# ArtoriasAbyssslayer/HashModNFFBanks-IDR

Hardware: AMD Instinct MI355X
Metric: rays/sec fwd+bwd (hash+SDF MLP) (higher is better)
Workload: dtype f32; 1 GPU; DTU-shaped synthetic uniform-sphere rays, MultiResHash L=16 T=2^19 F=2 (BASELINE.json configs[1]), full IDR training step (forward + IDRLoss + backward + clip + Adam), weights held at the geometric initialisation (lr = 0): the SURVEY.md 8(d) workload; grid_config=C2, rays_per_gpu=2048, global_rays=2048, parallelism=single GPU, world=1, ranks_seen=1, step=HIP-graph captured static-shape step

## Files before the change

hashmodnffbanks_idr_amd/_lib.py:

```python
import ctypes as C
import os

import torch

_PKG = os.path.dirname(os.path.abspath(__file__))
LIB_PATH = os.environ.get("HM_LIB_PATH") or os.path.join(_PKG, "libhashmod.so")
_lib = None

_p = C.c_void_p
_i64 = C.c_int64
_int = C.c_int

SIGNATURES = {
    "hm_version": (_int, []),
    "hm_last_error": (C.c_char_p, []),
    "hm_device_count": (_int, []),
    "hm_grid_desc_create": (_int, [_int, _int, _p, _p, _p, C.POINTER(_p)]),
    "hm_grid_desc_destroy": (None, [_p]),
    "hm_grid_embed_dim": (_int, [_p]),
    "hm_corner_ids": (_int, [_p, _int, _p, _i64, _p, _p, _p]),
    "hm_diag_gather_calib": (_int, [_p, _i64, _i64, _int, _int, _p, _p]),
    "hm_diag_mfma_f32_stream": (_int, [_int, _int, _p, _p]),
    "hm_encode_fwd": (_int, [_p, _p, _i64, _p, _p, _p, _i64, _int, _p]),
    "hm_encode_workspace_bytes": (_i64, [_p, _i64]),
# ... 2 lines not shown
    "hm_encode_bwd_workspace_bytes": (_i64, [_p, _i64]),
    "hm_encode_bwd_table_ws": (_int, [_p, _p, _i64, _p, _i64, _p, _int, _p, _i64, _p]),
    "hm_encode_rows": (_int, [_p, _p, _i64, _int, _p, _p, _p]),
    "hm_encode_bwd_table_sorted": (_int, [_p, _p, _p, _i64, _int, _p, _i64, _p, _p, _p]),
    "hm_sort_workspace_bytes": (_i64, [_i64]),
    "hm_sort_pairs_i32": (_int, [_p, _i64, _int, _p, _p, _p, _i64, _p]),
    "hm_encode_bwd_input": (_int, [_p, _p, _i64, _p, _p, _i64, _p, _p, _p]),
    "hm_encode_jvp": (_int, [_p, _p, _i64, _p, _p, _p, _i64, _p]),
    "hm_encode_bwd_table_jvp": (_int, [_p, _p, _i64, _p, _p, _i64, _p, _p]),
    "hm_fourier_bwd_input": (_int, [_p, _i64, _p, _int, _p, _i64, _p, _p]),
    "hm_fourier_bwd_input_bwd": (_int, [_p, _i64, _p, _int, _p, _i64, _p, _p, _p, _i64, _int, _p]),
    "hm_weight_norm_multi": (_int, [_int, _int, _p, _p]),
    "hm_rownorm": (_int, [_int, _p, _p, _p, _p, _p, _i64, _int, C.c_float, _p]),
    "hm_sine": (_int, [_int, _p, _p, _p, _p, _p, _i64, C.c_float, _p]),
    "hm_posenc": (_int, [_int, _p, _int, _int, _p, _i64, _p, _i64, _p, _p, _i64, _p, _i64, _p]),
    "hm_sdf_fwd": (_int, [_p, _p, _p, _i64, _p, _p, _p, _i64, _int, _int, _int, _p, _int, _p]),
    "hm_nffb_fwd": (_int, [_p, _p, _p, _i64, _p, _p, _p, _i64, _int, _p, _p]),
    "hm_sdf_fwd_emb": (_int, [_p, _p, _i64, _int, _i64, _p, _i64, _int, _int, _p, _int, _p]),
    "hm_sdf_net_fits": (_int, [_p, _int, _int]),
    "hm_diag_sdf_lds": (_int, [_p, _int, _int, _int, _p]),
    "hm_trace_workspace_bytes": (_i64, [_i64, _p]),
    "hm_trace_guard_clear": (_int, [_p, _i64, _p]),
    "hm_trace_guard_tolerances": (_int, [_p, _p]),
    "hm_trace_forward": (_int, [_p, _p, _p, _p, _int, _int, _p, _p, _p, _p, _p, _p, _i64, _i64, _p, _p, _p, _p, _p, _p,
                                _i64, _p, _p]),
    "hm_trace_workspace_bytes_nffb": (_i64, [_i64, _p, _int]),
    "hm_trace_forward_nffb": (_int, [_p, _p, _p, _p, _p, _int, _int, _p, _p, _p, _p, _p, _p, _i64, _i64, _p, _p, _p, _p,
                                     _p, _p, _i64, _p, _p]),
    "hm_pack_mlp_layer_bf16": (_int, [_p, _i64, _int, _int, _int, _p, _p]),
    "hm_sdf_fwd_bf16": (_int, [_p, _p, _p, _i64, _p, _p, _p, _i64, _int, _p, _i64, _p]),
    "hm_sdf_fwd_emb_bf16": (_int, [_p, _p, _i64, _int, _i64, _p, _i64, _p, _i64, _p]),
    "hm_pack_mlp_layer_split": (_int, [_p, _i64, _int, _int, _int, C.c_float, C.c_float, _int, _p, _p]),
    "hm_sdf_fwd_split": (_int, [_p, _p, _p, _i64, _p, _p, _p, _i64, _int, _p, _i64, _p]),
    "hm_sdf_fwd_emb_split": (_int, [_p, _p, _i64, _int, _i64, _p, _i64, _p, _i64, _p]),
    "hm_pack_mlp_layers": (_int, [_p, _int, _p]),
    "hm_pack_mlp_layer": (_int, [_p, _i64, _p, _int, _int, _int, _p, _p, _p, _p]),
    "hm_softplus": (_int, [_int, _p, _p, _p, _p, _p, _i64, C.c_float, C.c_float, _p]),
    "hm_sdf_head": (_int, [_int, _p, _i64, _i64, C.c_float, _p, _p, _p, _p, _p, _p]),
    "hm_colsum": (_int, [_p, _i64, _i64, _i64, _p, _p]),
    "hm_colsum_acc": (_int, [_p, _i64, _i64, _i64, _p, _p]),
    "hm_colsum_acc_multi": (_int, [_p, _int, _p]),
    "hm_copy2d_f32": (_int, [_p, _i64, _p, _i64, _i64, _i64, _p]),
    "hm_camera_rays": (_int, [_p, _p, _p, _i64, _i64, C.c_float, _p, _p, _p, _p, _p]),
    "hm_idr_loss": (_int, [_p, _p, _p, _p, _p, _i64, _p, _i64, C.c_float, C.c_float, C.c_float, _p, _p, _p, _p, _p]),
    "hm_idr_loss_dev": (_int, [_p, _p, _p, _p, _p, _i64, _p, _i64, _p, _p, _p, _p, _p, _p]),
    "hm_adam_scratch_floats": (_i64, [_p, _int]),
# ... 243 lines not shown
```

hashmodnffbanks_idr_amd/csrc/hm_sdf.hip:

```cpp
#include "hm_common.h"

#include <math.h>
#include <stdlib.h>

namespace {

#include "hm_sdf_common.h"
#include "hm_trace_dev.h"

#ifdef HM_SDF_PHASE_PROBE
__device__ unsigned long long hm_probe_ts[128];
#define HM_PROBE(i_)                                                                                  \
    do {                                                                                              \
        if (blockIdx.x == 0 && threadIdx.x == 0 && it == 1 && (i_) < 120) hm_probe_ts[(i_)] = wall_clock64(); \
        if (blockIdx.x == 0 && threadIdx.x == 0 && it == 1 && ((i_) == 0 || (i_) == 100))                 \
            hm_probe_ts[120 + ((i_) != 0)] = clock64();         \
    } while (0)
#define HM_PROBE_WAVES(base_)                                                                                  \
    do {                                                                                                       \
        if (blockIdx.x == 0 && (threadIdx.x & 63) == 0 && it == 1 && li == 2) hm_probe_ts[(base_) + (threadIdx.x >> 6)] = wall_clock64(); \
    } while (0)
#define HM_PROBE_S(i_)                                                                                \
    do {                                                                                              \
        if (blockIdx.x == 0 && threadIdx.x == 0 && (i_) < 120) hm_probe_ts[(i_)] = wall_clock64();   \
    } while (0)
#else
#define HM_PROBE(i_) do { } while (0)
#define HM_PROBE_WAVES(base_) do { } while (0)
#define HM_PROBE_S(i_) do { } while (0)
#endif

#include "hm_sdf_tile64.h"
#include "hm_sdf_split_tile.h"

__host__ __device__ inline SdfLds sdf_lds_small(const SdfNet &net, int E, int pts) {
    return sdf_lds(pts, 2, net.x_groups * pts * 4, 1, (E + 15) / 16 * 4 * pts * 4, kWaves);
}

template <int FRAC>
__global__ __launch_bounds__(kThreadsSdf, 2) void sdf_fwd_kernel(HmLevels lv, SdfNet net,
                                                                  const float *__restrict__ x, int64_t n,
                                                                  const float *__restrict__ table,
                                                                  const float *__restrict__ Bf,
                                                                  float *__restrict__ out, int64_t out_stride,
                                                                  int out_cols, const int32_t *__restrict__ n_dev, int64_t run_min,
                                                                  int64_t run_max, SdfFillArgs fa) {
    extern __shared__ __align__(16) float lds[];
    if (n_dev) n = min(n, (int64_t)max(*n_dev, 0));
    if (n < run_min || n > run_max) return;
    SdfFill fb = {nullptr, nullptr, 0, 0};
    if (fa.n_dev) {
        fb.x = fa.x;
        fb.out = fa.out;
        fb.n = max(*fa.n_dev, 0);
        if (fa.prev_dev)
            fb.tile0 = fill_quota(max(*fa.prev_dev, 0), fa.prev_grid, (fb.n + kPts - 1) / kPts, run_min);
// ... 400 lines not shown
                                                                          float *__restrict__ scan_out, int c_scan,
                                                                          int64_t scan_cap, int64_t scan_min,
                                                                          int64_t scan_hide, int c_prev1, int grid1,
                                                                          int c_prev2, int grid2) {
    extern __shared__ __align__(16) float lds[];
    const int64_t n_scan = min((int64_t)max(a.w.cnt[c_scan], 0), scan_cap);
    const int64_t n_sec = a.w.cnt[C_NSEC];
    if (n_sec > 0 && n_iters > 0) {
        const int pts = a.w.cnt[C_NSEL_PTS] >= scan_hide ? 16 : (n_sec <= m4_max ? 4 : (n_sec <= m8_max ? 8 : 16));
        secant_role<FRAC>(lv, net, table, Bf, a, n_iters, n_sec, pts, lds);
    }
    if (n_scan < scan_min) return;
    const int64_t tb = (n_scan + kPts - 1) / kPts;
    int64_t done = c_prev1 >= 0 ? fill_quota(max(a.w.cnt[c_prev1], 0), grid1, tb, scan_min) : 0;
    if (c_prev2 >= 0) done += fill_quota(max(a.w.cnt[c_prev2], 0), grid2, tb - done, scan_min);
    const int64_t skip = done * kPts;
    if (skip >= n_scan) return;
    const SdfFill none = {nullptr, nullptr, 0, 0};
    sdf64_run<FRAC, true>(lv, net, scan_x + skip * 3, n_scan - skip, table, Bf, scan_out + skip, 1, 1, lds,
                          reinterpret_cast<unsigned *>(a.w.cnt + C_TILE_CURSOR), none);
}

template <int KIND, int FRAC>
__global__ __launch_bounds__(kThreadsSdf, 2) void sdf_refine_scan_kernel(HmLevels lv, SdfNet net, SdfNet net_split,
                                                                          const float *__restrict__ table,
                                                                          const float *__restrict__ Bf, TraceArgs a,
                                                                          int c_ref, int64_t scan_off, int64_t scan_min) {
    extern __shared__ __align__(16) float lds[];
    __shared__ unsigned s_scan_tile;
    const int64_t n_ref = min((int64_t)max(a.w.cnt[c_ref], 0), a.w.cap);
    const int64_t n_scan = min((int64_t)max(a.w.cnt[C_NSEL_PTS], 0), a.w.cap);
    if (n_ref > 0) {
        const SdfFill none = {nullptr, nullptr, 0, 0};
        sdf64_run<FRAC, true>(lv, net, a.w.ref_pts, n_ref, table, Bf, a.w.ref_vals, 1, 1, lds,
                              reinterpret_cast<unsigned *>(a.w.cnt + C_XREF_CURSOR), none);
    }
    if (n_scan < scan_min) return;
    const int64_t n_tiles = (n_scan + kPS - 1) / kPS;
    unsigned *cursor = reinterpret_cast<unsigned *>(a.w.cnt + C_XSCAN_CURSOR);
    for (;;) {
        __syncthreads();
        if (threadIdx.x == 0) s_scan_tile = atomicAdd(cursor, 1u);
        __syncthreads();
        const int64_t tile = s_scan_tile;
        if (tile >= n_tiles) break;
        sdf_split_tile<KIND, FRAC>(lv, net_split, a.w.pts + scan_off * 3, n_scan, table, Bf, a.w.vals + scan_off, 1, lds,
                                   tile);
    }
}

static int sdf_net_fp32(const char *who, const HmLevels &lv, const hm_mlp_desc *mlp, int64_t emb_stride, SdfImage img,
                        SdfNet &net, bool *all_m16 = nullptr) {
    return sdf_net_from_desc(who, mlp, lv.E, emb_stride, img, 1, (lv.E + 7) / 8 * 2, false, net, all_m16);
}

constexpr size_t kLds16Max = 96 * 1024, kLds64Max = 160 * 1024, kLdsTrace = 64;

static int sdf_fp32_fits(const hm_mlp_desc *mlp, int E) {
    HmLevels lv = {};
    lv.E = E;
    SdfNet net;
    bool have16 = true;
    const int rc = sdf_net_fp32("hm_sdf_net_fits", lv, mlp, 0, kImgM16Optional, net, &have16);
    if (rc != HM_OK) return rc;
    HM_CHECK_ARG(sdf_lds64(net).bytes() + kLdsTrace <= kLds64Max, "hm_sdf_net_fits: network does not fit the 160 KB LDS tile");
    HM_CHECK_ARG(!have16 || sdf_lds_small(net, E, kPts16).bytes() + kLdsTrace <= kLds16Max,
                 "hm_sdf_net_fits: network does not fit the 16-point LDS tile");
    return HM_OK;
}

struct SmallTiles {
    int64_t m8_max, m4_max;
};
static SmallTiles sdf_small_tiles(int tile_points) {
    const int64_t kBig = (int64_t)1 << 62;
    if (tile_points == 16) return {0, 0};
    if (tile_points == 8) return {kBig, 0};
    if (tile_points == 4) return {kBig, kBig};
    return {kSdfTiny, kSdfMini};
}
static unsigned sdf_small_grid(int64_t n, SmallTiles t, int64_t cap) {
    int64_t tiles = t.m8_max >= n ? 0 : (n + kPts16 - 1) / kPts16;
    if (t.m8_max > 0) tiles = max(tiles, ((n < t.m8_max ? n : t.m8_max) + kPts8 - 1) / kPts8);
    if (t.m4_max > 0) tiles = max(tiles, ((n < t.m4_max ? n : t.m4_max) + 3) / 4);
    return (unsigned)(tiles < cap ? tiles : cap);
}

template <class F>
int sdf_dispatch(int mode, F &&f) {
    if (mode == kFracEmb) return f(std::integral_constant<int, kFracEmb>{});
    return hm_frac_dispatch(mode, f);
}

}

extern "C" {

int hm_diag_mfma_f32_stream(int workgroups, int iters, float *out, void *stream) {
    HM_CHECK_ARG(workgroups >= 1 && workgroups <= 65535 && iters >= 1 && out, "hm_diag_mfma_f32_stream: bad argument");
    hipLaunchKernelGGL(mfma_f32_stream_kernel, dim3((unsigned)workgroups), dim3(kThreadsSdf), 0, as_stream(stream), iters, out);
    HM_CHECK_LAUNCH("hm_diag_mfma_f32_stream");
    return HM_OK;
}

#ifdef HM_SDF_PHASE_PROBE
HM_API int hm_probe_read(unsigned long long *out, int n) {
    return hipMemcpyFromSymbol(out, HIP_SYMBOL(hm_probe_ts), sizeof(unsigned long long) * (size_t)(n < 128 ? n : 128)) == hipSuccess ? 0 : -1;
}
// ... 109 lines not shown
                        stream);
        if (rc != HM_OK) return rc;
    }
    const size_t lds16 = sdf_lds_small(net, desc->lv.E, kPts16).bytes(), lds64 = sdf_lds64(net).bytes();
    HM_CHECK_ARG(lds16 <= kLds16Max && lds64 <= kLds64Max - kLdsTrace, "hm_trace_scan_secant: network does not fit the LDS tiles");
    const size_t lds = lds16 > lds64 ? lds16 : lds64;
    static_assert(kTraceScanHide == 3 * 256 * kPts, "kTraceScanHide counts rounds of 64-point tiles");
    const int64_t scan_hide = kTraceScanHide;
    const int p1 = grid1 > 0 ? c_prev1 : -1, p2 = grid2 > 0 ? c_prev2 : -1;
    const SmallTiles t = sdf_small_tiles(0);
    return hm_frac_dispatch(frac_mode, [&](auto frac) {
        constexpr auto kernel = sdf_scan_secant_kernel<decltype(frac)::value>;
        const int rc = hm_allow_dynamic_lds<kernel>(160 * 1024 - 64);
        if (rc != HM_OK) return rc;
        hipLaunchKernelGGL(kernel, dim3(256), dim3(kThreadsSdf), lds, as_stream(stream), desc->lv, net, table, B_fourier, a,
                           n_iters, t.m8_max, t.m4_max, scan_x, scan_out, c_scan, scan_capacity,
                           (int64_t)(small_front ? kSdfSmall + 1 : 1), scan_hide, p1, grid1, p2, grid2);
        HM_CHECK_LAUNCH("hm_trace_scan_secant");
        return HM_OK;
    });
}

int hm_trace_refine_scan(const hm_grid_desc *desc, const hm_mlp_desc *mlp, const float *table, const float *B_fourier,
                         int frac_mode, const void *trace_args, int c_ref, int64_t scan_off, int64_t scan_capacity,
                         void *stream) {
    HM_CHECK_ARG(desc && mlp && table && B_fourier && trace_args, "hm_trace_refine_scan: NULL argument");
    HM_CHECK_ARG(frac_mode == HM_FRAC_REFERENCE || frac_mode == HM_FRAC_TRILINEAR, "hm_trace_refine_scan: bad frac_mode");
    HM_CHECK_ARG(c_ref >= 0 && c_ref < C_COUNT, "hm_trace_refine_scan: bad list counter");
    const TraceArgs &a = *static_cast<const TraceArgs *>(trace_args);
    static_assert(sizeof(HmLevels) + 2 * sizeof(SdfNet) + sizeof(TraceArgs) + 64 <= 4096, "kernel arguments exceed 4 KB");
    SdfNet net, net_split;
    size_t lds_split = 0;
    int rc = sdf_net_fp32("hm_trace_refine_scan", desc->lv, mlp, 0, kImgM16, net);
    if (rc == HM_OK) rc = sdf_split_net("hm_trace_refine_scan", desc->lv.E, mlp, 0, net_split, &lds_split);
    if (rc != HM_OK) return rc;
    if (a.n == 0) return HM_OK;
    HM_CHECK_ARG(a.w.pts && a.w.vals && a.w.ref_pts && a.w.ref_vals && a.w.cnt, "hm_trace_refine_scan: NULL workspace pointer");
    HM_CHECK_ARG(scan_off >= 0 && scan_capacity >= 0 && scan_capacity <= a.w.cap, "hm_trace_refine_scan: bad scan region");
    rc = hm_sdf_fwd(desc, mlp, a.w.pts + scan_off * 3, scan_capacity, table, B_fourier, a.w.vals + scan_off, 1, 1, frac_mode,
                    -1, a.w.cnt + C_NSEL_PTS, 0, stream);
    if (rc != HM_OK) return rc;
    const size_t lds64 = sdf_lds64(net).bytes();
    HM_CHECK_ARG(lds64 <= kLds64Max - kLdsTrace && lds_split <= kLds64Max - kLdsTrace,
                 "hm_trace_refine_scan: network does not fit the LDS tiles");
    const size_t lds = lds_split > lds64 ? lds_split : lds64;
    const int64_t tiles = (a.w.cap + 31) / 32;
    const unsigned grid = (unsigned)(tiles < 256 ? tiles : 256);
    const auto launch = [&](auto kind, auto frac) {
        constexpr auto kernel = sdf_refine_scan_kernel<decltype(kind)::value, decltype(frac)::value>;
        const int rc = hm_allow_dynamic_lds<kernel>(160 * 1024 - 64);
        if (rc != HM_OK) return rc;
        hipLaunchKernelGGL(kernel, dim3(grid), dim3(kThreadsSdf), lds, as_stream(stream), desc->lv, net, net_split, table,
                           B_fourier, a, c_ref, scan_off, (int64_t)kSdfSmall + 1);
        HM_CHECK_LAUNCH("hm_trace_refine_scan");
        return HM_OK;
    };
    return hm_frac_dispatch(frac_mode, [&](auto frac) {
        if (mlp->split_kind == HM_SPLIT_BF16X2) return launch(std::integral_constant<int, HM_SPLIT_BF16X2>{}, frac);
        return launch(std::integral_constant<int, HM_SPLIT_F16X2>{}, frac);
    });
}

static int sdf_fwd_impl(const HmLevels &lv, const hm_mlp_desc *mlp, const float *x, int64_t emb_stride, int64_t n,
                        const float *table, const float *B_fourier, float *out, int64_t out_stride, int out_cols,
                        int frac_mode, int tile_points, const int32_t *n_dev, int max_workgroups, void *stream,
                        const SdfFillArgs *fill, int *grid64_out) {
    HM_CHECK_ARG(n >= 0, "hm_sdf_fwd: n < 0");
    HM_CHECK_ARG(frac_mode == HM_FRAC_REFERENCE || frac_mode == HM_FRAC_TRILINEAR, "hm_sdf_fwd: bad frac_mode");
    HM_CHECK_ARG(tile_points == 0 || tile_points == 4 || tile_points == 8 || tile_points == 16 || tile_points == 64 ||
                     tile_points == -1,
                 "hm_sdf_fwd: tile_points must be -1, 0, 4, 8, 16 or 64");
    SdfNet net;
    bool have16 = true;
    {
        const int rc = sdf_net_fp32("hm_sdf_fwd", lv, mlp, emb_stride, kImgM16Optional, net, &have16);
        if (rc != HM_OK) return rc;
    }
    const int mode = emb_stride > 0 ? kFracEmb : frac_mode;
    const hm_mlp_layer &last = mlp->layer[mlp->n_layers - 1];
    HM_CHECK_ARG(out_cols == 1 || out_cols == last.out_dim, "hm_sdf_fwd: out_cols must be 1 or the last layer's out_dim");
    HM_CHECK_ARG(out_stride >= out_cols, "hm_sdf_fwd: out_stride < out_cols");
    HM_CHECK_ARG((tile_points != 16 && tile_points != 8 && tile_points != 4) || have16,
                 "hm_sdf_fwd: tile_points 4 / 8 / 16 need w_packed_m16 in every layer");
// ... 78 lines not shown
```

hashmodnffbanks_idr_amd/csrc/hm_trace.hip:

```cpp
#include "hm_common.h"

#include <stdlib.h>
#include <string.h>

extern "C" int hm_trace_march_tail(const hm_grid_desc *desc, const hm_mlp_desc *mlp, const float *table,
                                   const float *B_fourier, int frac_mode, int body16, const void *trace_args, int first,
                                   int rounds, void *stream);

extern "C" int hm_trace_secant_persistent(const hm_grid_desc *desc, const hm_mlp_desc *mlp, const float *table,
                                          const float *B_fourier, int frac_mode, int tile_points, const void *trace_args,
                                          int n_iters, int scan_rule, void *stream);

extern "C" int hm_trace_scan_secant(const hm_grid_desc *desc, const hm_mlp_desc *mlp, const float *table,
                                    const float *B_fourier, int frac_mode, const void *trace_args, int n_iters,
                                    const float *scan_x, float *scan_out, int64_t scan_capacity, int c_scan,
                                    int small_front, int c_prev1, int grid1, int c_prev2, int grid2, void *stream);

extern "C" int hm_trace_refine_scan(const hm_grid_desc *desc, const hm_mlp_desc *mlp, const float *table,
                                    const float *B_fourier, int frac_mode, const void *trace_args, int c_ref,
                                    int64_t scan_off, int64_t scan_capacity, void *stream);

extern "C" int hm_sdf_fwd_fill(const hm_grid_desc *desc, const hm_mlp_desc *mlp, const float *x, int64_t n,
                               const float *table, const float *B_fourier, float *out, int frac_mode, const int32_t *n_dev,
                               const float *x_fill, float *out_fill, const int32_t *n_fill_dev, const int32_t *prev_dev,
                               int prev_grid, int *grid64_out, void *stream);

namespace {

constexpr int kTB = 256;

#include "hm_trace_dev.h"

__global__ __launch_bounds__(kTB) void trace_init_kernel(TraceArgs a) {
    const int64_t i = (int64_t)blockIdx.x * kTB + threadIdx.x;
    if (i >= a.n) return;
    trace_init_ray(a, i, a.w.cnt + C_ROUND0, 0);
}

__global__ __launch_bounds__(kTB) void trace_advance_kernel(TraceArgs a, int round) {
    const int64_t i = (int64_t)blockIdx.x * kTB + threadIdx.x;
    if (i >= a.n) return;
    trace_advance_ray(a, i, a.w.cnt + C_ROUND0 + round, 0);
}
// ... 478 lines not shown
    a.w.cap = L.cap;
    a.w.ref_pts = reinterpret_cast<float *>(base + L.off_ref);
    a.w.ref_vals = a.w.ref_pts + 3 * (size_t)L.cap;
    a.w.ref_slot = reinterpret_cast<int32_t *>(a.w.ref_vals + (size_t)L.cap);
    a.w.guard = reinterpret_cast<int32_t *>(base);
    a.cam = cam_loc; a.dirs = ray_dirs; a.obj = object_mask; a.t_sphere = t_sphere; a.hit = hit_mask;
    a.fracs = sampler_fracs; a.steps_u = steps_u;
    a.out_pts = out_points; a.out_mask = out_net_mask; a.out_t = out_dists;
    a.n = n_rays; a.rays_per_image = rays_per_image;
    a.thr = cfg->sdf_threshold;
    for (int k = 0; k < 4; ++k) a.back[k] = (float)((1.0 - cfg->line_search_step) / (double)(1 << k));
    a.ls_iters = cfg->line_step_iters; a.max_it = cfg->sphere_tracing_iters; a.n_steps = cfg->n_steps;
    a.n_secant = cfg->n_secant_steps; a.training = cfg->training;
    a.head = (cfg->sampler_head >= 1 && cfg->sampler_head + 1 < cfg->n_steps) ? cfg->sampler_head : 0;
    a.tail_off = L.cap;
    const char *e_ov = getenv("HM_TRACE_OVERLAP");
    const bool overlap_ok = !(e_ov && atoi(e_ov) == 0);
    const bool overlap_shape = overlap_ok && cfg->training && !nffb && tile_points == 0 && cfg->n_secant_steps > 0 &&
                               n_rays <= kSdfSmall;
    const bool overlap = overlap_shape && !cfg->coarse_bf16;
    const bool sel_own = overlap || (guard && overlap_shape);
    a.sel_off = sel_own ? 2 * L.cap : -1;
    const bool cosched = guard && overlap_shape && !(e_ov && atoi(e_ov) == 1);

    hm_zero_u32_async(a.w.cnt, C_COUNT, st);
    const unsigned g_rays = (unsigned)((n_rays + kTB - 1) / kTB);
    const unsigned g_samp = (unsigned)((n_rays * cfg->n_steps + kTB - 1) / kTB);
    const unsigned g_rows = (unsigned)((n_rays + kGuardRows - 1) / kGuardRows);

    float *emb_ws = reinterpret_cast<float *>(base + L.off_emb);
    auto sdf = [&](int64_t capacity, const int32_t *n_dev) -> int {
        if (nffb) {
            const int rc = hm_nffb_fwd(desc, nffb, a.w.pts, capacity, table, B_fourier, emb_ws, emb_width, frac_mode,
                                       n_dev, stream);
            if (rc != HM_OK) return rc;
            return hm_sdf_fwd_emb(mlp, emb_ws, emb_width, emb_width, capacity, a.w.vals, 1, 1, tile_points, n_dev, 0,
                                  stream);
        }
        return hm_sdf_fwd(desc, mlp, a.w.pts, capacity, table, B_fourier, a.w.vals, 1, 1, frac_mode, tile_points, n_dev,
                          0, stream);
    };
    auto coarse = [&](int64_t off, int64_t capacity, const int32_t *n_dev) -> int {
        const float *p = a.w.pts + off * 3;
        float *v = a.w.vals + off;
        const int64_t run_min = kSdfSmall + 1;
        int rc;
// ... 73 lines not shown
    if (cfg->training) hipLaunchKernelGGL(tail_prepare_kernel, dim3(g_rays), dim3(kTB), 0, st, a);
    const int per_ray = a.head > 0 ? a.head + 1 : cfg->n_steps;
    const int c_first = a.head > 0 ? (int)C_HEAD_PTS : (int)C_NSAMP_PTS;
    hipLaunchKernelGGL(ray_samples_kernel, dim3((unsigned)((n_rays * per_ray + kTB - 1) / kTB)), dim3(kTB), 0, st, a,
                       a.w.list_samp, (int)C_NSAMP, c_first, a.w.t_s, a.w.t_e, sampler_fracs, -1, per_ray);
    if (cfg->training)
        hipLaunchKernelGGL(ray_samples_kernel, dim3(g_samp), dim3(kTB), 0, st, a, a.w.list_sel, (int)C_NSEL,
                           (int)C_NSEL_PTS, a.w.t_min, a.w.t_max, steps_u, sel_own ? -2 : c_first, cfg->n_steps);
    int grid_p1 = 0, grid_p2 = 0;
    if (overlap) {
        int rc = hm_sdf_fwd_fill(desc, mlp, a.w.pts, n_rays * cfg->n_steps, table, B_fourier, a.w.vals, frac_mode,
                                 a.w.cnt + c_first, a.w.pts + a.sel_off * 3, a.w.vals + a.sel_off, a.w.cnt + C_NSEL_PTS,
                                 nullptr, 0, &grid_p1, stream);
        if (rc != HM_OK) return rc;
    } else {
        const int c_samp = sel_own ? c_first : (int)C_BIG_PTS, c_sel = sel_own ? (int)C_NSEL_PTS : (int)C_BIG_PTS;
        int rc = coarse(0, n_rays * cfg->n_steps, a.w.cnt + c_samp);
        if (rc == HM_OK && sel_own && !cosched) rc = coarse(a.sel_off, n_rays * cfg->n_steps, a.w.cnt + c_sel);
        if (rc != HM_OK) return rc;
        if (cosched) {
            guard_noise(0, n_rays * cfg->n_steps, c_samp);
            hipLaunchKernelGGL(guard_select_sampler_kernel, dim3(g_rows), dim3(kTB), 0, st, a, 1, c_samp, -1, guard_min,
                               (int)C_GUARD_N1);
            rc = hm_trace_refine_scan(desc, mlp, table, B_fourier, frac_mode, &a, (int)C_GUARD_N1, a.sel_off,
                                      n_rays * cfg->n_steps, stream);
            if (rc != HM_OK) return rc;
            guard_patch((int)C_GUARD_N1);
        } else if (guard) {
            guard_noise(0, n_rays * cfg->n_steps, c_samp);
            if (sel_own) guard_noise(a.sel_off, n_rays * cfg->n_steps, c_sel);
            hipLaunchKernelGGL(guard_select_sampler_kernel, dim3(g_rows), dim3(kTB), 0, st, a, 1, c_samp, -1, guard_min,
                               (int)C_GUARD_N1);
            if (cfg->training)
                hipLaunchKernelGGL(guard_select_closest_kernel, dim3(g_rows), dim3(kTB), 0, st, a, c_sel, guard_min,
                                   (int)C_GUARD_N1);
            rc = guard_refine((int)C_GUARD_N1);
            if (rc != HM_OK) return rc;
        }
    }
    if (cfg->training && !overlap && !cosched) hipLaunchKernelGGL(closest_reduce_kernel, dim3(g_rays), dim3(kTB), 0, st, a);
    if (a.head > 0) {
        hipLaunchKernelGGL(sampler_head_kernel, dim3(g_rays), dim3(kTB), 0, st, a);
        hipLaunchKernelGGL(sampler_tail_points_kernel, dim3(g_samp), dim3(kTB), 0, st, a);
        int rc = overlap ? hm_sdf_fwd_fill(desc, mlp, a.w.pts + a.tail_off * 3, n_rays * (cfg->n_steps - a.head - 1), table,
                                           B_fourier, a.w.vals + a.tail_off, frac_mode, a.w.cnt + C_TAIL_PTS,
                                           a.w.pts + a.sel_off * 3, a.w.vals + a.sel_off, a.w.cnt + C_NSEL_PTS,
                                           a.w.cnt + c_first, grid_p1, &grid_p2, stream)
                         : coarse(a.tail_off, n_rays * (cfg->n_steps - a.head - 1), a.w.cnt + C_TAIL_PTS);
        if (rc != HM_OK) return rc;
        if (guard) {
            guard_noise(a.tail_off, n_rays * (cfg->n_steps - a.head - 1), (int)C_TAIL_PTS);
            hipLaunchKernelGGL(guard_select_sampler_kernel, dim3(g_rows), dim3(kTB), 0, st, a, 2, (int)C_TAIL_PTS,
                               sel_own ? c_first : (int)C_BIG_PTS, guard_min, (int)C_GUARD_N2);
            rc = guard_refine((int)C_GUARD_N2);
            if (rc != HM_OK) return rc;
        }
    }
    hipLaunchKernelGGL(sampler_reduce_kernel, dim3(g_rays), dim3(kTB), 0, st, a);
    if (cfg->n_secant_steps > 0) {
        hipLaunchKernelGGL(secant_points_kernel, dim3(g_rays), dim3(kTB), 0, st, a);
        if (overlap) {
            const int rc = hm_trace_scan_secant(desc, mlp, table, B_fourier, frac_mode, &a, cfg->n_secant_steps,
                                                a.w.pts + a.sel_off * 3, a.w.vals + a.sel_off, n_rays * cfg->n_steps,
                                                (int)C_NSEL_PTS, 1, c_first, grid_p1, (int)C_TAIL_PTS, grid_p2, stream);
            if (rc != HM_OK) return rc;
            hipLaunchKernelGGL(closest_reduce_kernel, dim3(g_rays), dim3(kTB), 0, st, a);
        } else if (cosched) {
            guard_noise(a.sel_off, n_rays * cfg->n_steps, (int)C_NSEL_PTS);
            hipLaunchKernelGGL(guard_select_closest_kernel, dim3(g_rows), dim3(kTB), 0, st, a, (int)C_NSEL_PTS, guard_min,
                               (int)C_GUARD_NC);
            const int rc = hm_trace_scan_secant(desc, mlp, table, B_fourier, frac_mode, &a, cfg->n_secant_steps, a.w.ref_pts,
                                                a.w.ref_vals, L.cap, (int)C_GUARD_NC, 0, -1, 0, -1, 0, stream);
            if (rc != HM_OK) return rc;
            guard_patch((int)C_GUARD_NC);
            hipLaunchKernelGGL(closest_reduce_kernel, dim3(g_rays), dim3(kTB), 0, st, a);
        } else if (!nffb && (tile_points == 0 || tile_points == 4 || tile_points == 8 || tile_points == 16) &&
            (tile_points != 0 || n_rays <= kSdfSmall)) {
            const int rc = hm_trace_secant_persistent(desc, mlp, table, B_fourier, frac_mode, tile_points, &a,
                                                      cfg->n_secant_steps, sel_own ? 1 : 0, stream);
            if (rc != HM_OK) return rc;
        } else {
            for (int s = 0; s < cfg->n_secant_steps; ++s) {
                int rc = sdf(n_rays, a.w.cnt + C_NSEC);
                if (rc != HM_OK) return rc;
                hipLaunchKernelGGL(secant_advance_kernel, dim3(g_rays), dim3(kTB), 0, st, a,
                                   s == cfg->n_secant_steps - 1 ? 1 : 0);
            }
        }
    }
// ... 11 lines not shown
```

hashmodnffbanks_idr_amd/csrc/hm_trace_dev.h:

```cpp
#pragma once

enum : int32_t {
    C_ROUND0 = 0,
    C_NSAMP = 64,
    C_NSAMP_PTS = 65,
    C_NSEC = 66,
    C_NSEL = 67,
    C_NSEL_PTS = 68,
    C_ANY_LIVE = 69,
    C_EVALS = 70,
    C_UNFINISHED = 71,
    C_BIG_PTS = 73,
    C_NONFINITE = 72,
    C_NSAMP2 = 74,
    C_HEAD_PTS = 75,
    C_TAIL_PTS = 76,
    C_TILE_CURSOR = 77,
    C_GUARD_REFINED = 78,
    C_GUARD_MAXDEV = 79,
    C_GUARD_N1 = 80,
    C_GUARD_N2 = 81,
    C_GUARD_NC = 82,
    C_XREF_CURSOR = 83,
    C_XSCAN_CURSOR = 84,
    C_COUNT = 96
};

constexpr float kGuardTau = 1.52587890625e-05f;
constexpr float kGuardTrip = kGuardTau * 0.25f;
constexpr int32_t kGuardTripped = 0x47554152;

constexpr int64_t kTraceScanHide = 3 * 256 * 64;

enum : uint8_t { ST_WAIT_FIRST = 1, ST_WAIT_MARCH = 2, ST_WAIT_LS = 3, ST_DONE = 4 };

struct TraceWs {
    float *t_s, *t_e, *t_min, *t_max, *cur_s, *cur_e, *nxt_s, *nxt_e;
    float *z_lo, *z_hi, *v_lo, *v_hi, *z;
    int32_t *slot_s, *slot_e, *list_samp, *list_sec, *list_sel;
    int32_t *tail_slot;
    uint8_t *live_s, *live_e, *stage, *it, *k, *is_samp;
    float *pts;
    float *vals;
    int32_t *cnt;
    int64_t cap;
    float *ref_pts;
    float *ref_vals;
    int32_t *ref_slot;
    int32_t *guard;
};

struct TraceArgs {
    TraceWs w;
    const float *cam;
    const float *dirs;
// ... 147 lines not shown
```

include/hashmod.h:

```cpp
#ifndef HASHMOD_H
#define HASHMOD_H

#include <stdint.h>

#ifdef __cplusplus
extern "C" {
#endif

#if defined(__GNUC__)
#define HM_API __attribute__((visibility("default")))
#else
#define HM_API
#endif

#define HM_MAX_LEVELS 32
#define HM_MAX_LAYERS 16

#define HM_FRAC_REFERENCE 0
#define HM_FRAC_TRILINEAR 1

#define HM_OK 0
#define HM_ERR_INVALID (-1)
#define HM_ERR_HIP (-2)

// ... 134 lines not shown
    const float *out_w, *out_b;
    const float *style_w, *style_b;
} hm_nffb_desc;
HM_API int hm_nffb_fwd(const hm_grid_desc *desc, const hm_nffb_desc *nf, const float *x, int64_t n, const float *table,
                       const float *B_fourier, float *out, int64_t out_stride, int frac_mode, const int32_t *n_dev,
                       void *stream);

typedef struct hm_trace_cfg {
    float object_bounding_sphere;
    float sdf_threshold;
    double line_search_step;
    int32_t line_step_iters;
    int32_t sphere_tracing_iters;
    int32_t n_steps;
    int32_t n_secant_steps;
    int32_t training;
    int32_t coarse_bf16;
    int32_t sampler_head;
} hm_trace_cfg;

HM_API int64_t hm_trace_workspace_bytes(int64_t n_rays, const hm_trace_cfg *cfg);
HM_API int hm_trace_guard_clear(void *workspace, int64_t workspace_bytes, void *stream);
HM_API int hm_trace_guard_tolerances(float *tau, float *tau_trip);
HM_API int hm_trace_forward(const hm_grid_desc *desc, const hm_mlp_desc *mlp, const float *table,
                            const float *B_fourier, int frac_mode, int tile_points, const hm_trace_cfg *cfg,
                            const float *cam_loc, const float *ray_dirs, const uint8_t *object_mask,
                            const float *t_sphere, const uint8_t *hit_mask, int64_t n_rays, int64_t rays_per_image,
                            const float *sampler_fracs, const float *steps_u, float *out_points,
                            uint8_t *out_net_mask, float *out_dists, void *workspace, int64_t workspace_bytes,
                            int32_t *stats_out, void *stream);

HM_API int64_t hm_trace_workspace_bytes_nffb(int64_t n_rays, const hm_trace_cfg *cfg, int n_levels);
HM_API int hm_trace_forward_nffb(const hm_grid_desc *desc, const hm_nffb_desc *nffb, const hm_mlp_desc *mlp,
                                 const float *table, const float *B_fourier, int frac_mode, int tile_points,
                                 const hm_trace_cfg *cfg, const float *cam_loc, const float *ray_dirs,
                                 const uint8_t *object_mask, const float *t_sphere, const uint8_t *hit_mask,
                                 int64_t n_rays, int64_t rays_per_image, const float *sampler_fracs,
                                 const float *steps_u, float *out_points, uint8_t *out_net_mask, float *out_dists,
                                 void *workspace, int64_t workspace_bytes, int32_t *stats_out, void *stream);

HM_API int hm_gemm_f32(int transA, int transB, int64_t M, int64_t N, int64_t K, const float *A, int64_t lda,
                       const float *B, int64_t ldb, const float *bias, float *C, int64_t ldc, int accumulate,
                       void *stream);

enum { HM_EPI_NONE = 0, HM_EPI_SOFTPLUS = 1, HM_EPI_S1MUL = 2, HM_EPI_ADJOINT = 3, HM_EPI_RELU = 4, HM_EPI_RELUMASK = 5 };
typedef struct hm_gemm_epilogue {
// ... 260 lines not shown
```

Measured before the change: 292,400 rays/s.

## Pool split-precision scan tiles across refine launches and secant kernel

Splits the split-precision scan tile work into three quota ranges. Each range goes to a different place: idle workgroups of the first refine launch, idle workgroups of the second guard-refine launch, or leftover capacity beside the secant role in a new combined secant+scan kernel. The aim is to fill idle compute units during the small refine and secant phases instead of running the scan as separate dedicated work. The cost is a more complex quota heuristic that depends on a fixed chain-tiles-per-secant-iteration constant. It also adds extra cursors and a changed launch order that could unbalance work or add tail latency.

```diff
diff --git a/hashmodnffbanks_idr_amd/_lib.py b/hashmodnffbanks_idr_amd/_lib.py
--- a/hashmodnffbanks_idr_amd/_lib.py
+++ b/hashmodnffbanks_idr_amd/_lib.py
@@ -48,6 +48,7 @@
     "hm_trace_workspace_bytes": (_i64, [_i64, _p]),
     "hm_trace_guard_clear": (_int, [_p, _i64, _p]),
     "hm_trace_guard_tolerances": (_int, [_p, _p]),
+    "hm_trace_scan_pool_plan": (_int, [_i64, _i64, _i64, _int, _int, _i64, _int, _i64, _p, _p]),
     "hm_trace_forward": (_int, [_p, _p, _p, _p, _int, _int, _p, _p, _p, _p, _p, _p, _i64, _i64, _p, _p, _p, _p, _p, _p,
                                 _i64, _p, _p]),
     "hm_trace_workspace_bytes_nffb": (_i64, [_i64, _p, _int]),
diff --git a/hashmodnffbanks_idr_amd/csrc/hm_scan_pool.h b/hashmodnffbanks_idr_amd/csrc/hm_scan_pool.h
--- /dev/null
+++ b/hashmodnffbanks_idr_amd/csrc/hm_scan_pool.h
@@ -0,0 +1,39 @@
+#pragma once
+
+struct ScanPool {
+    int64_t first[3], quota[3];
+};
+
+__host__ __device__ inline int64_t sdf64_busy_workgroups(int64_t n, int64_t grid) {
+    if (n <= 0) return 0;
+    if (n / kPts >= grid) return grid;
+    const int64_t step = n <= grid * 32 ? 32 : kPts;
+    const int64_t tiles = (n + step - 1) / step;
+    return tiles < grid ? tiles : grid;
+}
+
+__host__ __device__ inline ScanPool scan_pool_quota(int64_t n_scan, int64_t n_ref1, int64_t n_ref2, int two_x,
+                                                    int64_t grid_x, int64_t n_sec_bound, int64_t chain_tiles) {
+    const int64_t tiles = n_scan > kSdfSmall ? (n_scan + kPS - 1) / kPS : 0;
+    int64_t capacity = 0;
+    if (n_sec_bound > 0 && chain_tiles > 0) {
+        const int pts = n_scan >= kTraceScanHide ? 16 : (n_sec_bound <= kSdfMini ? 4 : (n_sec_bound <= kSdfTiny ? 8 : 16));
+        const int64_t sec_tiles = (n_sec_bound + pts - 1) / pts;
+        capacity = (256 - (sec_tiles < 256 ? sec_tiles : 256)) * chain_tiles;
+    }
+    const int64_t over = tiles > capacity ? tiles - capacity : 0;
+    const int64_t idle1 = grid_x - sdf64_busy_workgroups(n_ref1, grid_x);
+    const int64_t idle2 = grid_x - sdf64_busy_workgroups(n_ref2, grid_x);
+    ScanPool p;
+    const int64_t want1 = two_x ? idle1 : (idle1 > over ? idle1 : over);
+    p.quota[0] = want1 < tiles ? want1 : tiles;
+    const int64_t left = tiles - p.quota[0];
+    const int64_t over2 = over > p.quota[0] ? over - p.quota[0] : 0;
+    const int64_t want2 = two_x ? (idle2 > over2 ? idle2 : over2) : 0;
+    p.quota[1] = want2 < left ? want2 : left;
+    p.quota[2] = left - p.quota[1];
+    p.first[0] = 0;
+    p.first[1] = p.quota[0];
+    p.first[2] = p.quota[0] + p.quota[1];
+    return p;
+}
diff --git a/hashmodnffbanks_idr_amd/csrc/hm_sdf.hip b/hashmodnffbanks_idr_amd/csrc/hm_sdf.hip
--- a/hashmodnffbanks_idr_amd/csrc/hm_sdf.hip
+++ b/hashmodnffbanks_idr_amd/csrc/hm_sdf.hip
@@ -32,6 +32,7 @@
 
 #include "hm_sdf_tile64.h"
 #include "hm_sdf_split_tile.h"
+#include "hm_scan_pool.h"
 
 __host__ __device__ inline SdfLds sdf_lds_small(const SdfNet &net, int E, int pts) {
     return sdf_lds(pts, 2, net.x_groups * pts * 4, 1, (E + 15) / 16 * 4 * pts * 4, kWaves);
@@ -478,31 +479,64 @@
 }
 
 template <int KIND, int FRAC>
+__device__ __forceinline__ void split_scan_range(const HmLevels &lv, const SdfNet &net_split, const float *__restrict__ table,
+                                                 const float *__restrict__ Bf, const TraceArgs &a, int64_t scan_off,
+                                                 int64_t n_scan, int64_t first, int64_t quota, unsigned *cursor, float *lds) {
+    __shared__ unsigned s_scan_tile;
+    if (quota <= 0) return;
+    for (;;) {
+        __syncthreads();
+        if (threadIdx.x == 0) s_scan_tile = atomicAdd(cursor, 1u);
+        __syncthreads();
+        const int64_t k = s_scan_tile;
+        if (k >= quota) break;
+        sdf_split_tile<KIND, FRAC>(lv, net_split, a.w.pts + scan_off * 3, n_scan, table, Bf, a.w.vals + scan_off, 1, lds,
+                                   first + k);
+    }
+}
+
+template <int KIND, int FRAC>
 __global__ __launch_bounds__(kThreadsSdf, 2) void sdf_refine_scan_kernel(HmLevels lv, SdfNet net, SdfNet net_split,
                                                                           const float *__restrict__ table,
                                                                           const float *__restrict__ Bf, TraceArgs a,
-                                                                          int c_ref, int64_t scan_off, int64_t scan_min) {
+                                                                          int c_ref1, int c_ref2, int which,
+                                                                          int64_t scan_off, int64_t chain_tiles) {
     extern __shared__ __align__(16) float lds[];
-    __shared__ unsigned s_scan_tile;
-    const int64_t n_ref = min((int64_t)max(a.w.cnt[c_ref], 0), a.w.cap);
+    const int64_t n_ref1 = min((int64_t)max(a.w.cnt[c_ref1], 0), a.w.cap);
+    const int64_t n_ref2 = which ? min((int64_t)max(a.w.cnt[c_ref2], 0), a.w.cap) : 0;
+    const int64_t n_ref = which ? n_ref2 : n_ref1;
     const int64_t n_scan = min((int64_t)max(a.w.cnt[C_NSEL_PTS], 0), a.w.cap);
     if (n_ref > 0) {
         const SdfFill none = {nullptr, nullptr, 0, 0};
         sdf64_run<FRAC, true>(lv, net, a.w.ref_pts, n_ref, table, Bf, a.w.ref_vals, 1, 1, lds,
-                              reinterpret_cast<unsigned *>(a.w.cnt + C_XREF_CURSOR), none);
-    }
-    if (n_scan < scan_min) return;
-    const int64_t n_tiles = (n_scan + kPS - 1) / kPS;
-    unsigned *cursor = reinterpret_cast<unsigned *>(a.w.cnt + C_XSCAN_CURSOR);
-    for (;;) {
-        __syncthreads();
-        if (threadIdx.x == 0) s_scan_tile = atomicAdd(cursor, 1u);
-        __syncthreads();
-        const int64_t tile = s_scan_tile;
-        if (tile >= n_tiles) break;
-        sdf_split_tile<KIND, FRAC>(lv, net_split, a.w.pts + scan_off * 3, n_scan, table, Bf, a.w.vals + scan_off, 1, lds,
-                                   tile);
-    }
+                              reinterpret_cast<unsigned *>(a.w.cnt + (which ? C_XREF2_CURSOR : C_XREF_CURSOR)), none);
+    }
+    const ScanPool p = scan_pool_quota(n_scan, n_ref1, n_ref2, c_ref2 >= 0, gridDim.x, a.w.cnt[C_NSAMP], chain_tiles);
+    split_scan_range<KIND, FRAC>(lv, net_split, table, Bf, a, scan_off, n_scan, which ? p.first[1] : p.first[0],
+                                 which ? p.quota[1] : p.quota[0],
+                                 reinterpret_cast<unsigned *>(a.w.cnt + (which ? C_XSCAN2_CURSOR : C_XSCAN_CURSOR)), lds);
+}
+
+template <int KIND, int FRAC>
+__global__ __launch_bounds__(kThreadsSdf, 2) void sdf_split_scan_secant_kernel(HmLevels lv, SdfNet net, SdfNet net_split,
+                                                                                const float *__restrict__ table,
+                                                                                const float *__restrict__ Bf, TraceArgs a,
+                                                                                int n_iters, int64_t m8_max, int64_t m4_max,
+                                                                                int64_t scan_hide, int c_ref1, int c_ref2,
+                                                                                int grid_x, int64_t scan_off,
+                                                                                int64_t chain_tiles) {
+    extern __shared__ __align__(16) float lds[];
+    const int64_t n_sec = a.w.cnt[C_NSEC];
+    if (n_sec > 0 && n_iters > 0) {
+        const int pts = a.w.cnt[C_NSEL_PTS] >= scan_hide ? 16 : (n_sec <= m4_max ? 4 : (n_sec <= m8_max ? 8 : 16));
+        secant_role<FRAC>(lv, net, table, Bf, a, n_iters, n_sec, pts, lds);
+    }
+    const int64_t n_scan = min((int64_t)max(a.w.cnt[C_NSEL_PTS], 0), a.w.cap);
+    const int64_t n_ref1 = min((int64_t)max(a.w.cnt[c_ref1], 0), a.w.cap);
+    const int64_t n_ref2 = c_ref2 >= 0 ? min((int64_t)max(a.w.cnt[c_ref2], 0), a.w.cap) : 0;
+    const ScanPool p = scan_pool_quota(n_scan, n_ref1, n_ref2, c_ref2 >= 0, grid_x, a.w.cnt[C_NSAMP], chain_tiles);
+    split_scan_range<KIND, FRAC>(lv, net_split, table, Bf, a, scan_off, n_scan, p.first[2], p.quota[2],
+                                 reinterpret_cast<unsigned *>(a.w.cnt + C_YSCAN_CURSOR), lds);
 }
 
 static int sdf_net_fp32(const char *who, const HmLevels &lv, const hm_mlp_desc *mlp, int64_t emb_stride, SdfImage img,
@@ -540,6 +574,11 @@
     if (t.m8_max > 0) tiles = max(tiles, ((n < t.m8_max ? n : t.m8_max) + kPts8 - 1) / kPts8);
     if (t.m4_max > 0) tiles = max(tiles, ((n < t.m4_max ? n : t.m4_max) + 3) / 4);
     return (unsigned)(tiles < cap ? tiles : cap);
+}
+
+static unsigned refine_scan_grid(int64_t cap) {
+    const int64_t tiles = (cap + 31) / 32;
+    return (unsigned)(tiles < 256 ? tiles : 256);
 }
 
 template <class F>
@@ -695,11 +734,13 @@
 }
 
 int hm_trace_refine_scan(const hm_grid_desc *desc, const hm_mlp_desc *mlp, const float *table, const float *B_fourier,
-                         int frac_mode, const void *trace_args, int c_ref, int64_t scan_off, int64_t scan_capacity,
-                         void *stream) {
+                         int frac_mode, const void *trace_args, int c_ref1, int c_ref2, int which, int64_t scan_off,
+                         int64_t scan_capacity, int64_t chain_tiles, void *stream) {
     HM_CHECK_ARG(desc && mlp && table && B_fourier && trace_args, "hm_trace_refine_scan: NULL argument");
     HM_CHECK_ARG(frac_mode == HM_FRAC_REFERENCE || frac_mode == HM_FRAC_TRILINEAR, "hm_trace_refine_scan: bad frac_mode");
-    HM_CHECK_ARG(c_ref >= 0 && c_ref < C_COUNT, "hm_trace_refine_scan: bad list counter");
+    HM_CHECK_ARG(c_ref1 >= 0 && c_ref1 < C_COUNT && c_ref2 < C_COUNT, "hm_trace_refine_scan: bad list counter");
+    HM_CHECK_ARG((which == 0 || which == 1) && (which == 0 || c_ref2 >= 0) && chain_tiles >= 0,
+                 "hm_trace_refine_scan: bad launch index / chain capacity");
     const TraceArgs &a = *static_cast<const TraceArgs *>(trace_args);
     static_assert(sizeof(HmLevels) + 2 * sizeof(SdfNet) + sizeof(TraceArgs) + 64 <= 4096, "kernel arguments exceed 4 KB");
     SdfNet net, net_split;
@@ -710,21 +751,22 @@
     if (a.n == 0) return HM_OK;
     HM_CHECK_ARG(a.w.pts && a.w.vals && a.w.ref_pts && a.w.ref_vals && a.w.cnt, "hm_trace_refine_scan: NULL workspace pointer");
     HM_CHECK_ARG(scan_off >= 0 && scan_capacity >= 0 && scan_capacity <= a.w.cap, "hm_trace_refine_scan: bad scan region");
-    rc = hm_sdf_fwd(desc, mlp, a.w.pts + scan_off * 3, scan_capacity, table, B_fourier, a.w.vals + scan_off, 1, 1, frac_mode,
-                    -1, a.w.cnt + C_NSEL_PTS, 0, stream);
-    if (rc != HM_OK) return rc;
+    if (which == 0) {
+        rc = hm_sdf_fwd(desc, mlp, a.w.pts + scan_off * 3, scan_capacity, table, B_fourier, a.w.vals + scan_off, 1, 1,
+                        frac_mode, -1, a.w.cnt + C_NSEL_PTS, 0, stream);
+        if (rc != HM_OK) return rc;
+    }
     const size_t lds64 = sdf_lds64(net).bytes();
     HM_CHECK_ARG(lds64 <= kLds64Max - kLdsTrace && lds_split <= kLds64Max - kLdsTrace,
                  "hm_trace_refine_scan: network does not fit the LDS tiles");
     const size_t lds = lds_split > lds64 ? lds_split : lds64;
-    const int64_t tiles = (a.w.cap + 31) / 32;
-    const unsigned grid = (unsigned)(tiles < 256 ? tiles : 256);
+    const unsigned grid = refine_scan_grid(a.w.cap);
     const auto launch = [&](auto kind, auto frac) {
         constexpr auto kernel = sdf_refine_scan_kernel<decltype(kind)::value, decltype(frac)::value>;
         const int rc = hm_allow_dynamic_lds<kernel>(160 * 1024 - 64);
         if (rc != HM_OK) return rc;
         hipLaunchKernelGGL(kernel, dim3(grid), dim3(kThreadsSdf), lds, as_stream(stream), desc->lv, net, net_split, table,
-                           B_fourier, a, c_ref, scan_off, (int64_t)kSdfSmall + 1);
+                           B_fourier, a, c_ref1, c_ref2, which, scan_off, chain_tiles);
         HM_CHECK_LAUNCH("hm_trace_refine_scan");
         return HM_OK;
     };
@@ -732,6 +774,59 @@
         if (mlp->split_kind == HM_SPLIT_BF16X2) return launch(std::integral_constant<int, HM_SPLIT_BF16X2>{}, frac);
         return launch(std::integral_constant<int, HM_SPLIT_F16X2>{}, frac);
     });
+}
+
+int hm_trace_split_scan_secant(const hm_grid_desc *desc, const hm_mlp_desc *mlp, const float *table,
+                               const float *B_fourier, int frac_mode, const void *trace_args, int n_iters, int c_ref1,
+                               int c_ref2, int64_t scan_off, int64_t scan_capacity, int64_t chain_tiles, void *stream) {
+    HM_CHECK_ARG(desc && mlp && table && B_fourier && trace_args, "hm_trace_split_scan_secant: NULL argument");
+    HM_CHECK_ARG(frac_mode == HM_FRAC_REFERENCE || frac_mode == HM_FRAC_TRILINEAR,
+                 "hm_trace_split_scan_secant: bad frac_mode");
+    HM_CHECK_ARG(c_ref1 >= 0 && c_ref1 < C_COUNT && c_ref2 < C_COUNT && chain_tiles >= 0,
+                 "hm_trace_split_scan_secant: bad list counter / chain capacity");
+    const TraceArgs &a = *static_cast<const TraceArgs *>(trace_args);
+    SdfNet net, net_split;
+    size_t lds_split = 0;
+    int rc = sdf_net_fp32("hm_trace_split_scan_secant", desc->lv, mlp, 0, kImgM16, net);
+    if (rc == HM_OK) rc = sdf_split_net("hm_trace_split_scan_secant", desc->lv.E, mlp, 0, net_split, &lds_split);
+    if (rc != HM_OK) return rc;
+    if (a.n == 0) return HM_OK;
+    HM_CHECK_ARG(a.w.pts && a.w.vals && a.w.cnt, "hm_trace_split_scan_secant: NULL workspace pointer");
+    HM_CHECK_ARG(scan_off >= 0 && scan_capacity >= 0 && scan_capacity <= a.w.cap, "hm_trace_split_scan_secant: bad scan region");
+    const size_t lds16 = sdf_lds_small(net, desc->lv.E, kPts16).bytes();
+    HM_CHECK_ARG(lds16 <= kLds16Max && lds_split <= kLds64Max - kLdsTrace,
+                 "hm_trace_split_scan_secant: network does not fit the LDS tiles");
+    const size_t lds = lds16 > lds_split ? lds16 : lds_split;
+    const int grid_x = (int)refine_scan_grid(a.w.cap);
+    const SmallTiles t = sdf_small_tiles(0);
+    const auto launch = [&](auto kind, auto frac) {
+        constexpr auto kernel = sdf_split_scan_secant_kernel<decltype(kind)::value, decltype(frac)::value>;
+        const int rc = hm_allow_dynamic_lds<kernel>(160 * 1024 - 64);
+        if (rc != HM_OK) return rc;
+        hipLaunchKernelGGL(kernel, dim3(256), dim3(kThreadsSdf), lds, as_stream(stream), desc->lv, net, net_split, table,
+                           B_fourier, a, n_iters, t.m8_max, t.m4_max, (int64_t)kTraceScanHide, c_ref1, c_ref2, grid_x,
+                           scan_off, chain_tiles);
+        HM_CHECK_LAUNCH("hm_trace_split_scan_secant");
+        return HM_OK;
+    };
+    return hm_frac_dispatch(frac_mode, [&](auto frac) {
+        if (mlp->split_kind == HM_SPLIT_BF16X2) return launch(std::integral_constant<int, HM_SPLIT_BF16X2>{}, frac);
+        return launch(std::integral_constant<int, HM_SPLIT_F16X2>{}, frac);
+    });
+}
+
+int hm_trace_scan_pool_plan(int64_t n_scan, int64_t n_ref1, int64_t n_ref2, int two_x, int grid_x, int64_t n_sec_bound,
+                            int n_iters, int64_t chain_tiles, int64_t *first, int64_t *quota) {
+    HM_CHECK_ARG(n_scan >= 0 && n_ref1 >= 0 && n_ref2 >= 0 && grid_x >= 1 && grid_x <= 256 && n_sec_bound >= 0 &&
+                     n_iters >= 0 && chain_tiles >= -1 && first && quota,
+                 "hm_trace_scan_pool_plan: bad argument");
+    const ScanPool p = scan_pool_quota(n_scan, n_ref1, n_ref2, two_x != 0, grid_x, n_sec_bound,
+                                       trace_chain_tiles(n_iters, chain_tiles));
+    for (int k = 0; k < 3; ++k) {
+        first[k] = p.first[k];
+        quota[k] = p.quota[k];
+    }
+    return HM_OK;
 }
 
 static int sdf_fwd_impl(const HmLevels &lv, const hm_mlp_desc *mlp, const float *x, int64_t emb_stride, int64_t n,
diff --git a/hashmodnffbanks_idr_amd/csrc/hm_trace.hip b/hashmodnffbanks_idr_amd/csrc/hm_trace.hip
--- a/hashmodnffbanks_idr_amd/csrc/hm_trace.hip
+++ b/hashmodnffbanks_idr_amd/csrc/hm_trace.hip
@@ -17,8 +17,13 @@
                                     int small_front, int c_prev1, int grid1, int c_prev2, int grid2, void *stream);
 
 extern "C" int hm_trace_refine_scan(const hm_grid_desc *desc, const hm_mlp_desc *mlp, const float *table,
-                                    const float *B_fourier, int frac_mode, const void *trace_args, int c_ref,
-                                    int64_t scan_off, int64_t scan_capacity, void *stream);
+                                    const float *B_fourier, int frac_mode, const void *trace_args, int c_ref1, int c_ref2,
+                                    int which, int64_t scan_off, int64_t scan_capacity, int64_t chain_tiles, void *stream);
+
+extern "C" int hm_trace_split_scan_secant(const hm_grid_desc *desc, const hm_mlp_desc *mlp, const float *table,
+                                          const float *B_fourier, int frac_mode, const void *trace_args, int n_iters,
+                                          int c_ref1, int c_ref2, int64_t scan_off, int64_t scan_capacity,
+                                          int64_t chain_tiles, void *stream);
 
 extern "C" int hm_sdf_fwd_fill(const hm_grid_desc *desc, const hm_mlp_desc *mlp, const float *x, int64_t n,
                                const float *table, const float *B_fourier, float *out, int frac_mode, const int32_t *n_dev,
@@ -543,6 +548,10 @@
     const bool sel_own = overlap || (guard && overlap_shape);
     a.sel_off = sel_own ? 2 * L.cap : -1;
     const bool cosched = guard && overlap_shape && !(e_ov && atoi(e_ov) == 1);
+    const bool pool = cosched && !(e_ov && atoi(e_ov) == 2);
+    const char *e_ct = getenv("HM_TRACE_POOL_CHAIN_TILES");
+    const int64_t chain_tiles = pool ? trace_chain_tiles(cfg->n_secant_steps, (e_ct && atoi(e_ct) >= 0) ? atoi(e_ct) : -1) : 0;
+    const int c_ref2 = (pool && a.head > 0) ? (int)C_GUARD_N2 : -1;
 
     hm_zero_u32_async(a.w.cnt, C_COUNT, st);
     const unsigned g_rays = (unsigned)((n_rays + kTB - 1) / kTB);
@@ -662,8 +671,8 @@
             guard_noise(0, n_rays * cfg->n_steps, c_samp);
             hipLaunchKernelGGL(guard_select_sampler_kernel, dim3(g_rows), dim3(kTB), 0, st, a, 1, c_samp, -1, guard_min,
                                (int)C_GUARD_N1);
-            rc = hm_trace_refine_scan(desc, mlp, table, B_fourier, frac_mode, &a, (int)C_GUARD_N1, a.sel_off,
-                                      n_rays * cfg->n_steps, stream);
+            rc = hm_trace_refine_scan(desc, mlp, table, B_fourier, frac_mode, &a, (int)C_GUARD_N1, c_ref2, 0, a.sel_off,
+                                      n_rays * cfg->n_steps, chain_tiles, stream);
             if (rc != HM_OK) return rc;
             guard_patch((int)C_GUARD_N1);
         } else if (guard) {
@@ -692,7 +701,13 @@
             guard_noise(a.tail_off, n_rays * (cfg->n_steps - a.head - 1), (int)C_TAIL_PTS);
             hipLaunchKernelGGL(guard_select_sampler_kernel, dim3(g_rows), dim3(kTB), 0, st, a, 2, (int)C_TAIL_PTS,
                                sel_own ? c_first : (int)C_BIG_PTS, guard_min, (int)C_GUARD_N2);
-            rc = guard_refine((int)C_GUARD_N2);
+            if (c_ref2 >= 0) {
+                rc = hm_trace_refine_scan(desc, mlp, table, B_fourier, frac_mode, &a, (int)C_GUARD_N1, c_ref2, 1, a.sel_off,
+                                          n_rays * cfg->n_steps, chain_tiles, stream);
+                guard_patch(c_ref2);
+            } else {
+                rc = guard_refine((int)C_GUARD_N2);
+            }
             if (rc != HM_OK) return rc;
         }
     }
@@ -705,6 +720,17 @@
                                                 (int)C_NSEL_PTS, 1, c_first, grid_p1, (int)C_TAIL_PTS, grid_p2, stream);
             if (rc != HM_OK) return rc;
             hipLaunchKernelGGL(closest_reduce_kernel, dim3(g_rays), dim3(kTB), 0, st, a);
+        } else if (pool) {
+            int rc = hm_trace_split_scan_secant(desc, mlp, table, B_fourier, frac_mode, &a, cfg->n_secant_steps,
+                                                (int)C_GUARD_N1, c_ref2, a.sel_off, n_rays * cfg->n_steps, chain_tiles,
+                                                stream);
+            if (rc != HM_OK) return rc;
+            guard_noise(a.sel_off, n_rays * cfg->n_steps, (int)C_NSEL_PTS);
+            hipLaunchKernelGGL(guard_select_closest_kernel, dim3(g_rows), dim3(kTB), 0, st, a, (int)C_NSEL_PTS, guard_min,
+                               (int)C_GUARD_NC);
+            rc = guard_refine((int)C_GUARD_NC);
+            if (rc != HM_OK) return rc;
+            hipLaunchKernelGGL(closest_reduce_kernel, dim3(g_rays), dim3(kTB), 0, st, a);
         } else if (cosched) {
             guard_noise(a.sel_off, n_rays * cfg->n_steps, (int)C_NSEL_PTS);
             hipLaunchKernelGGL(guard_select_closest_kernel, dim3(g_rows), dim3(kTB), 0, st, a, (int)C_NSEL_PTS, guard_min,
diff --git a/hashmodnffbanks_idr_amd/csrc/hm_trace_dev.h b/hashmodnffbanks_idr_amd/csrc/hm_trace_dev.h
--- a/hashmodnffbanks_idr_amd/csrc/hm_trace_dev.h
+++ b/hashmodnffbanks_idr_amd/csrc/hm_trace_dev.h
@@ -23,6 +23,9 @@
     C_GUARD_NC = 82,
     C_XREF_CURSOR = 83,
     C_XSCAN_CURSOR = 84,
+    C_XREF2_CURSOR = 85,
+    C_XSCAN2_CURSOR = 86,
+    C_YSCAN_CURSOR = 87,
     C_COUNT = 96
 };
 
@@ -31,6 +34,12 @@
 constexpr int32_t kGuardTripped = 0x47554152;
 
 constexpr int64_t kTraceScanHide = 3 * 256 * 64;
+
+constexpr int64_t kScanTilesPerSecantIterPermille = 875;
+inline int64_t trace_chain_tiles(int n_iters, int64_t given) {
+    if (n_iters <= 0) return 0;
+    return given >= 0 ? given : n_iters * kScanTilesPerSecantIterPermille / 1000;
+}
 
 enum : uint8_t { ST_WAIT_FIRST = 1, ST_WAIT_MARCH = 2, ST_WAIT_LS = 3, ST_DONE = 4 };
 
diff --git a/include/hashmod.h b/include/hashmod.h
--- a/include/hashmod.h
+++ b/include/hashmod.h
@@ -180,6 +180,8 @@
 HM_API int64_t hm_trace_workspace_bytes(int64_t n_rays, const hm_trace_cfg *cfg);
 HM_API int hm_trace_guard_clear(void *workspace, int64_t workspace_bytes, void *stream);
 HM_API int hm_trace_guard_tolerances(float *tau, float *tau_trip);
+HM_API int hm_trace_scan_pool_plan(int64_t n_scan, int64_t n_ref1, int64_t n_ref2, int two_x, int grid_x,
+                                   int64_t n_sec_bound, int n_iters, int64_t chain_tiles, int64_t *first, int64_t *quota);
 HM_API int hm_trace_forward(const hm_grid_desc *desc, const hm_mlp_desc *mlp, const float *table,
                             const float *B_fourier, int frac_mode, int tile_points, const hm_trace_cfg *cfg,
                             const float *cam_loc, const float *ray_dirs, const uint8_t *object_mask,
```

After: 309,800 rays/s (median of 6 runs). 1.06x the previous value.
